# zscole/adversarial-spec

Hardware: AMD Instinct MI355X
Metric: critiques/sec (debate round: 8192-token spec prefill + 512-token critique decode + RCCL consensus all-gather) (higher is better)
Workload: dtype bf16; 1 GPU; model=llama-3-8b, opponents=3, opponents_per_gpu=3, global_batch=3, seq_len=8192, parallelism=opponent-parallel dp1

## Files before the change

### adversarial_spec_amd/models/llama.py

```python

from __future__ import annotations

import math
import os
from dataclasses import dataclass
from typing import Optional

import torch

if torch.cuda.is_available():
    try:
        torch.backends.cuda.preferred_blas_library("cublas")
    except Exception:
        pass

from .. import ops
from ..ops import torch_ref
from .config import LlamaConfig


@dataclass
class QuantW:
    q: torch.Tensor
    s: torch.Tensor
# ... 338 lines not shown

        def proj(x, L_, Qd, name, out):
            qw = Qd.get(name) if Qd is not None else None
            if qw is not None:
                ops.gemv_fp8(x, qw.q, qw.s, W.x8, W.xs, out.view(1, -1))
                return out
            return ops.gemv(x, getattr(L_, name), out=out)

        fused = self.tp is None or self.tp.size == 1
        fused_f8 = (
            fused and fp8 and self.lm_head_q is not None
            and all(
                q.get(f) is not None for q in self.layers_q
                for f in self.FP8_PROJECTIONS
            )
        )

        fused_bf = fused and not fp8

        torch.index_select(self.embed, 0, W.tok_long, out=W.resid)
        if not (fused_bf or fused_f8):
            ops.rmsnorm(W.resid, self.layers[0].attn_norm, c.norm_eps,
                        out=W.normed)
        for i, L in enumerate(self.layers):
            Qd = self.layers_q[i] if fp8 else None
            if fused_f8:
                qw = Qd.get("wqkv")
                if _FP8_LDS:
                    ops.gemv_fp8_norm(W.resid, L.attn_norm, qw.q, qw.s,
                                      c.norm_eps, W.qkv)
                else:
                    ops.quant_norm_fp8(W.resid, L.attn_norm, W.x8, W.xs,
                                       c.norm_eps)
                    ops.gemv_fp8_q(W.x8, W.xs, qw.q, qw.s, W.qkv)
            elif fused_bf:
                ops.gemv_norm(W.resid, L.attn_norm, L.wqkv, c.norm_eps,
                              out=W.qkv)
            else:
                proj(W.normed, L, Qd, "wqkv", W.qkv)
            q = W.qkv[:, : h * hd].view(1, h, hd)
            k = W.qkv[:, h * hd : (h + kh) * hd].view(1, kh, hd)
            v = W.qkv[:, (h + kh) * hd :].view(1, kh, hd)
            ops.rope_kv(q, k, v, self.cos, self.sin, cache.k[i], cache.v[i],
                        cache.page_table, 0, pos_state=pos_state)
            ops.attn_decode_paged(
                q[0], cache.k[i], cache.v[i], cache.page_table,
                max_seq_bound, self.scale, pos_state=pos_state, out=W.attn,
                identity=cache.identity, split_blocks=self.split_blocks,
            )
            if fused_f8:
                gw = Qd.get("w_gate_up")
                if _FP8_LDS:
                    ops.gemv_fp8_resl(W.attn.view(1, h * hd),
                                      Qd.get("wo").q, Qd.get("wo").s,
                                      W.resid)
                    ops.gemv_fp8_gateup_norm(W.resid, L.mlp_norm, gw.q,
                                             gw.s, c.norm_eps, W.act)
                    ops.gemv_fp8_resl(W.act, Qd.get("w_down").q,
                                      Qd.get("w_down").s, W.resid)
                else:
                    ops.gemv_fp8_res(W.attn.view(1, h * hd),
                                     Qd.get("wo").q, Qd.get("wo").s,
                                     W.x8, W.xs, W.resid)
                    ops.quant_norm_fp8(W.resid, L.mlp_norm, W.x8, W.xs,
                                       c.norm_eps)
                    ops.gemv_fp8_gateup(W.x8, W.xs, gw.q, gw.s, W.act)
                    ops.gemv_fp8_res(W.act, Qd.get("w_down").q,
# ... 53 lines not shown
```

### adversarial_spec_amd/ops/__init__.py

```python

from __future__ import annotations

import os
from typing import Optional, Tuple

import torch

from . import torch_ref

_hip = None
_hip_err: Optional[str] = None


def _load_hip():
    global _hip, _hip_err
    if _hip is not None or _hip_err is not None:
        return _hip
    try:
        from . import _advspec_hip

        _hip = _advspec_hip
    except ImportError as e:
        _hip_err = str(e)
    return _hip
# ... 154 lines not shown
    f = w_gate_up.shape[0] // 2
    gu = x @ w_gate_up.t()
    y = torch_ref.swiglu(gu[..., :f], gu[..., f:])
    out.copy_(y.reshape(out.shape))
    return out


def _rms_ref(x: torch.Tensor, eps: float) -> torch.Tensor:
    xf = x.float()
    return torch.rsqrt(xf.pow(2).mean(-1, keepdim=True) + eps)


def gemv_norm(x: torch.Tensor, wln: torch.Tensor, w: torch.Tensor, eps: float,
              out: Optional[torch.Tensor] = None) -> torch.Tensor:
    if _on_gpu(x):
        return _require_hip().gemv_norm(x, wln, w, eps, out)
    y = ((x.float() * _rms_ref(x, eps) * wln.float()) @ w.float().t()).to(x.dtype)
    if out is not None:
        out.copy_(y.reshape(out.shape))
        return out
    return y


def gemv_res(x: torch.Tensor, w: torch.Tensor, resid: torch.Tensor) -> torch.Tensor:
    if _on_gpu(x):
        _require_hip().gemv_res(x, w, resid)
        return resid
    resid.add_((x.float() @ w.float().t()).to(resid.dtype).reshape(resid.shape))
    return resid


def gemv_gateup_norm(x: torch.Tensor, wln: torch.Tensor, w_gate_up: torch.Tensor,
                     eps: float, out: torch.Tensor) -> torch.Tensor:
    if _on_gpu(x):
        _require_hip().gemv_gateup_norm(x, wln, w_gate_up, eps, out)
        return out
    normed = (x.float() * _rms_ref(x, eps) * wln.float()).to(x.dtype)
    return gemv_gateup(normed, w_gate_up, out)


def gemm(x: torch.Tensor, w: torch.Tensor) -> torch.Tensor:
    if _on_gpu(x):
        return _require_hip().gemm(x, w)
    return x @ w.t()


# ... 133 lines not shown
```

### adversarial_spec_amd/ops/hip/attention.hip

```cpp

#include "common.h"

#define MAXG 8

template <int LPP>
DEVINL float group_reduce_sum(float v) {
#pragma unroll
  for (int off = LPP / 2; off > 0; off >>= 1) v += __shfl_xor(v, off, WAVE);
  return v;
}


#define DTILE 64

template <int LPP, int MG, bool IDENT>
__global__ void __launch_bounds__(256) attn_decode_split_kernel(
    const ushort_t *__restrict__ q,
    const ushort_t *__restrict__ kc, const ushort_t *__restrict__ vc,
    const int *__restrict__ page_table, int seq_len, float scale,
    int kh, int group, int hd, int page, int split_len,
    float *__restrict__ ws_m, float *__restrict__ ws_l,
    float *__restrict__ ws_acc, const int *__restrict__ pos_ptr,
    ushort_t *__restrict__ out) {
  if (pos_ptr) seq_len = *pos_ptr + 1;
// ... 157 lines not shown
      if (lane < LPP) {
        const float inv = (l[gi] > 0.f) ? 1.0f / l[gi] : 0.f;
        bf16x8 o;
#pragma unroll
        for (int j = 0; j < 8; ++j) o.u[j] = f32_to_bf16(acc[gi][j] * inv);
        ((bf16x8 *)(out + (size_t)(g * group + gq) * hd))[sl] = o;
      }
    } else {
      const size_t base = ((size_t)g * n_splits + split) * group + gq;
      if (lane == 0) {
        ws_m[base] = m[gi];
        ws_l[base] = l[gi];
      }
      if (lane < LPP) {
#pragma unroll
        for (int j = 0; j < 8; ++j)
          ws_acc[base * hd + sl * 8 + j] = acc[gi][j];
      }
    }
  }
}


extern "C" __global__ void __launch_bounds__(256)
attn_decode_combine_kernel(const float *__restrict__ ws_m,
                           const float *__restrict__ ws_l,
                           const float *__restrict__ ws_acc,
                           ushort_t *__restrict__ out, int n_splits,
                           int group, int hd) {
  const int h = blockIdx.x;
  const int g = h / group, gi = h % group;
  const int dd = blockIdx.y * 64 + (threadIdx.x & (WAVE - 1));
  const int sg = threadIdx.x / WAVE;
  if (dd >= hd) return;

  __shared__ float red[4];
  __shared__ float redL[4];

  float m = -INFINITY;
  {
    float m4[4] = {-INFINITY, -INFINITY, -INFINITY, -INFINITY};
    int s = sg;
    for (; s + 12 < n_splits; s += 16) {
#pragma unroll
      for (int u = 0; u < 4; ++u)
        m4[u] = fmaxf(m4[u],
                      ws_m[((size_t)g * n_splits + s + 4 * u) * group + gi]);
    }
    for (; s < n_splits; s += 4)
      m4[0] = fmaxf(m4[0], ws_m[((size_t)g * n_splits + s) * group + gi]);
    m = fmaxf(fmaxf(m4[0], m4[1]), fmaxf(m4[2], m4[3]));
  }
  if ((threadIdx.x & (WAVE - 1)) == 0) red[sg] = m;
  __syncthreads();
  const float M = fmaxf(fmaxf(red[0], red[1]), fmaxf(red[2], red[3]));

  float L = 0.f, Au[4] = {0.f, 0.f, 0.f, 0.f};
  int s = sg;
  for (; s + 12 < n_splits; s += 16) {
#pragma unroll
    for (int u = 0; u < 4; ++u) {
      const size_t b = ((size_t)g * n_splits + s + 4 * u) * group + gi;
      const float mw = ws_m[b];
      const float sc = (mw == -INFINITY) ? 0.f : exp2f(mw - M);
      L += ws_l[b] * sc;
      Au[u] += ws_acc[b * hd + dd] * sc;
    }
  }
  for (; s < n_splits; s += 4) {
    const size_t b = ((size_t)g * n_splits + s) * group + gi;
    const float mw = ws_m[b];
    const float sc = (mw == -INFINITY) ? 0.f : exp2f(mw - M);
    L += ws_l[b] * sc;
    Au[0] += ws_acc[b * hd + dd] * sc;
  }
  float A = (Au[0] + Au[1]) + (Au[2] + Au[3]);

  __shared__ float accs[4][64];
  accs[sg][threadIdx.x & (WAVE - 1)] = A;
  if ((threadIdx.x & (WAVE - 1)) == 0) redL[sg] = L;
  __syncthreads();
  if (sg == 0) {
    A = accs[0][threadIdx.x] + accs[1][threadIdx.x] + accs[2][threadIdx.x] +
        accs[3][threadIdx.x];
    L = redL[0] + redL[1] + redL[2] + redL[3];
    out[(size_t)h * hd + dd] = f32_to_bf16(L > 0.f ? A / L : 0.f);
  }
}


template <int LPP>
__global__ void __launch_bounds__(256) attn_prefill_simple_kernel(
    const ushort_t *__restrict__ q, const ushort_t *__restrict__ k,
    const ushort_t *__restrict__ v, ushort_t *__restrict__ out,
    int tq, int tk, int kv_offset, float scale, int hq, int kh, int hd,
    int causal) {
  const int h = blockIdx.x;
// ... 110 lines not shown
```

### adversarial_spec_amd/ops/hip/bindings.hip

```cpp

#include <torch/extension.h>
#include <c10/hip/HIPStream.h>
#include <hip/hip_runtime.h>

#include <cstdlib>
#include <mutex>
#include <unordered_map>
#include <vector>

using ushort_t = unsigned short;

extern "C" {
void launch_attn_decode_split(const ushort_t*, const ushort_t*, const ushort_t*,
                              const int*, int, float, int, int, int, int, int,
                              int, float*, float*, float*, const int*,
                              ushort_t*, int, hipStream_t);
void launch_attn_prefill_simple(const ushort_t*, const ushort_t*, const ushort_t*,
                                ushort_t*, int, int, int, float, int, int, int,
                                int, hipStream_t);
void launch_attn_prefill_mfma(const ushort_t*, const ushort_t*, const ushort_t*,
                              ushort_t*, int, int, int, float, int, int, int,
                              hipStream_t, int* ok);
void launch_attn_prefill_mfma_abl(const ushort_t*, const ushort_t*,
                                  const ushort_t*, ushort_t*, int, int, float,
// ... 1 lines not shown
__global__ void mfma_probe_16x16x32(const ushort_t*, const ushort_t*, float*);
__global__ void rmsnorm_kernel(const ushort_t*, const ushort_t*, ushort_t*, int, float);
__global__ void add_rmsnorm_kernel(const ushort_t*, const ushort_t*, const ushort_t*,
                                   ushort_t*, ushort_t*, int, float);
__global__ void rope_kernel(ushort_t*, ushort_t*, const float*, const float*,
                            int, int, int, int, int, long, long, const int*);
__global__ void swiglu_kernel(const ushort_t*, const ushort_t*, ushort_t*, int, int, int);
__global__ void kv_write_kernel(const ushort_t*, const ushort_t*, ushort_t*, ushort_t*,
                                const int*, int, int, int, int, int, const int*);
__global__ void rope_kv_kernel(ushort_t*, ushort_t*, const ushort_t*,
                               const float*, const float*, ushort_t*, ushort_t*,
                               const int*, int, int, int, int, int, long, long,
                               long, int, const int*);
__global__ void sample_kernel(const ushort_t*, int, float, uint32_t, int*);
__global__ void sample_state_kernel(const ushort_t*, int, const float*,
                                    uint32_t*, int*, const int*, long long*);
__global__ void bump_kernel(int*, int*);
void launch_gemv(const ushort_t*, const ushort_t*, ushort_t*, int, int,
                 hipStream_t);
void launch_gemv_gateup(const ushort_t*, const ushort_t*, ushort_t*, int, int,
                        hipStream_t);
void launch_gemv_norm(const ushort_t*, const ushort_t*, const ushort_t*,
                      ushort_t*, int, int, float, hipStream_t);
void launch_gemv_res(const ushort_t*, const ushort_t*, ushort_t*, int, int,
                     hipStream_t);
void launch_gemv_gateup_norm(const ushort_t*, const ushort_t*, const ushort_t*,
                             ushort_t*, int, int, float, hipStream_t);
void launch_gemm(const ushort_t*, const ushort_t*, ushort_t*, int, int, int,
                 hipStream_t);
void launch_gemm256(const ushort_t*, const ushort_t*, ushort_t*, int, int, int,
                    hipStream_t);
void launch_gemm_fp8(const uint8_t*, const float*, const uint8_t*, const float*,
                     ushort_t*, int, int, int, hipStream_t);
void launch_gemm_fp8_256(const uint8_t*, const float*, const uint8_t*,
                         const float*, ushort_t*, int, int, int, hipStream_t);
void launch_quant_norm_fp8(const ushort_t*, const ushort_t*, uint8_t*, float*,
                           int, float, hipStream_t);
void launch_gemv_fp8_norm(const ushort_t*, const ushort_t*, const uint8_t*,
                          const float*, ushort_t*, int, int, float,
                          hipStream_t);
void launch_gemv_fp8_resl(const ushort_t*, const uint8_t*, const float*,
                          ushort_t*, int, int, hipStream_t);
void launch_gemv_fp8_gateup_norm(const ushort_t*, const ushort_t*,
                                 const uint8_t*, const float*, ushort_t*,
                                 int, int, float, hipStream_t);
void launch_gemv_fp8_res(const uint8_t*, const float*, const uint8_t*,
// ... 359 lines not shown

torch::Tensor gemv_norm(torch::Tensor x, torch::Tensor wln, torch::Tensor w,
                        double eps, c10::optional<torch::Tensor> out_opt) {
  CHECK_BF16_CUDA(x);
  CHECK_BF16_CUDA(wln);
  CHECK_BF16_CUDA(w);
  TORCH_CHECK(w.dim() == 2 && w.is_contiguous());
  const int N = w.size(0), K = w.size(1);
  TORCH_CHECK((long)x.numel() == (long)K, "gemv_norm: x numel == K");
  TORCH_CHECK((long)wln.numel() == (long)K, "gemv_norm: wln numel == K");
  TORCH_CHECK(K % 8 == 0, "gemv_norm: K % 8 == 0");
  TORCH_CHECK(K <= 32768, "gemv_norm: LDS xl staging caps K at 32768");
  auto xc = x.contiguous();
  auto lc = wln.contiguous();
  auto y = out_opt.has_value()
               ? *out_opt
               : torch::empty(x.dim() == 2 ? std::vector<int64_t>{1, N}
                                           : std::vector<int64_t>{N},
                              x.options());
  TORCH_CHECK((long)y.numel() == (long)N, "gemv_norm: out numel == N");
  launch_gemv_norm(uptr(xc), uptr(lc), uptr(w), uptr_mut(y), K, N,
                   (float)eps, cur_stream());
  return y;
}

void gemv_res(torch::Tensor x, torch::Tensor w, torch::Tensor resid) {
  CHECK_BF16_CUDA(x);
  CHECK_BF16_CUDA(w);
  CHECK_BF16_CUDA(resid);
  TORCH_CHECK(w.dim() == 2 && w.is_contiguous());
  const int N = w.size(0), K = w.size(1);
  TORCH_CHECK((long)x.numel() == (long)K && K % 8 == 0);
  TORCH_CHECK((long)resid.numel() == (long)N, "gemv_res: resid numel == N");
  TORCH_CHECK(resid.is_contiguous());
  TORCH_CHECK(N <= 8192, "gemv_res: w32 kernel only (hidden <= 8192)");
  auto xc = x.contiguous();
  launch_gemv_res(uptr(xc), uptr(w), uptr_mut(resid), K, N, cur_stream());
}

void gemv_gateup_norm(torch::Tensor x, torch::Tensor wln, torch::Tensor w,
                      double eps, torch::Tensor act) {
  CHECK_BF16_CUDA(x);
  CHECK_BF16_CUDA(wln);
  CHECK_BF16_CUDA(w);
  CHECK_BF16_CUDA(act);
  TORCH_CHECK(w.dim() == 2 && w.is_contiguous());
// ... 311 lines not shown
  m.def("gemm_variant", &gemm_variant, "force GEMM kernel 128/256 (A/B)");
  m.def("gemm_fp8", &gemm_fp8, "fp8 e4m3 MFMA GEMM (rowwise scales)");
  m.def("gemv_fp8", &gemv_fp8, "fp8 decode GEMV (rowwise scales)");
  m.def("quant_norm_fp8", &quant_norm_fp8,
        "fused rmsnorm + rowwise e4m3 quantize (fp8 decode fusion)");
  m.def("gemv_fp8_q", &gemv_fp8_q, "pre-quantized fp8 decode GEMV");
  m.def("gemv_fp8_res", &gemv_fp8_res,
        "fp8 GEMV with residual-add epilogue (fp8 decode fusion)");
  m.def("gemv_fp8_gateup", &gemv_fp8_gateup,
        "pre-quantized fp8 gate_up GEMV + SwiGLU (fp8 decode fusion)");
  m.def("gemv_fp8_norm", &gemv_fp8_norm,
        "rmsnorm + quantize + fp8 GEMV, one launch (LDS-staged)");
  m.def("gemv_fp8_resl", &gemv_fp8_resl,
        "quantize + fp8 GEMV + residual epilogue, one launch (LDS-staged)");
  m.def("gemv_fp8_gateup_norm", &gemv_fp8_gateup_norm,
        "rmsnorm + quantize + fp8 gate_up GEMV + SwiGLU, one launch");
  m.def("quant_fp8", &quant_fp8, "rowwise bf16 -> e4m3 quantizer");
  m.def("mfma_rate", &mfma_rate, "MFMA issue-rate microbench (bf16/fp8)");
  m.def("rope_inplace_ds", &rope_inplace_ds, "graph-mode RoPE (device pos)");
  m.def("rope_kv", &rope_kv, "fused RoPE + paged KV scatter",
        py::arg("q"), py::arg("k"), py::arg("v"), py::arg("cost"),
        py::arg("sint"), py::arg("kc"), py::arg("vc"), py::arg("page_table"),
        py::arg("pos0"), py::arg("pos_state") = py::none());
  m.def("kv_write_ds", &kv_write_ds, "graph-mode KV scatter (device pos)");
  m.def("attn_decode_paged_ds", &attn_decode_paged_ds,
        "graph-mode paged decode attention (device pos)",
        py::arg("q"), py::arg("kc"), py::arg("vc"), py::arg("page_table"),
        py::arg("pos_state"), py::arg("max_seq"), py::arg("scale"),
        py::arg("out") = py::none(), py::arg("identity") = false,
        py::arg("split_blocks") = 0);
  m.def("sample_state", &sample_state, "graph-mode on-device sampling");
  m.def("bump", &bump, "graph-mode pos/step bump");
  m.def("ws_release", &ws_release,
        "drop decode-attention scratch for a dead KV cache");
}
```

### adversarial_spec_amd/ops/hip/common.h

```cpp
#pragma once

#include <hip/hip_runtime.h>
#include <hip/hip_bf16.h>
#include <stdint.h>

#define WAVE 64
#define DEVINL __device__ __forceinline__

typedef unsigned short ushort_t;


DEVINL float bf16_to_f32(ushort_t u) {
  union { uint32_t i; float f; } c;
  c.i = ((uint32_t)u) << 16;
  return c.f;
}

DEVINL ushort_t f32_to_bf16(float f) {
  union { uint32_t i; float f; } c;
  c.f = f;
  uint32_t lsb = (c.i >> 16) & 1u;
  c.i += 0x7fffu + lsb;
  return (ushort_t)(c.i >> 16);
}

struct bf16x8 { ushort_t u[8]; };
struct f32x8  { float v[8]; };

DEVINL f32x8 unpack8(const bf16x8 &p) {
  f32x8 r;
#pragma unroll
  for (int i = 0; i < 8; ++i) r.v[i] = bf16_to_f32(p.u[i]);
  return r;
}

DEVINL bf16x8 pack8(const f32x8 &p) {
  bf16x8 r;
#pragma unroll
  for (int i = 0; i < 8; ++i) r.u[i] = f32_to_bf16(p.v[i]);
  return r;
}

typedef __attribute__((__vector_size__(2 * sizeof(short)))) short bf16x2v_;

DEVINL float dot8_bf16(const bf16x8 &a, const bf16x8 &b, float acc) {
  const bf16x2v_ *ap = (const bf16x2v_ *)&a;
// ... 66 lines not shown
```

### adversarial_spec_amd/ops/hip/elementwise.hip

```cpp

#include "common.h"


extern "C" __global__ void __launch_bounds__(1024)
rmsnorm_kernel(const ushort_t *__restrict__ x, const ushort_t *__restrict__ w,
               ushort_t *__restrict__ y, int d, float eps) {
  __shared__ float scratch[16];
  const int row = blockIdx.x;
  const ushort_t *xr = x + (size_t)row * d;
  ushort_t *yr = y + (size_t)row * d;
  const int nvec = d / 8;

  float ss = 0.f;
  for (int i = threadIdx.x; i < nvec; i += blockDim.x) {
    f32x8 v = unpack8(((const bf16x8 *)xr)[i]);
#pragma unroll
    for (int j = 0; j < 8; ++j) ss += v.v[j] * v.v[j];
  }
  ss = block_reduce_sum(ss, scratch);
  const float inv = rsqrtf(ss / d + eps);

  for (int i = threadIdx.x; i < nvec; i += blockDim.x) {
    f32x8 v = unpack8(((const bf16x8 *)xr)[i]);
    f32x8 ww = unpack8(((const bf16x8 *)w)[i]);
// ... 103 lines not shown
    const int vh = slot - hq - hk;
    const bf16x8 *src =
        (const bf16x8 *)(v + (size_t)tok * v_rstride + (size_t)vh * hd);
    bf16x8 *dst = (bf16x8 *)(vc + cache_row + (size_t)vh * hd);
    for (int i = lane; i < hd / 8; i += WAVE) dst[i] = src[i];
    return;
  }

  const bool is_q = slot < hq;
  ushort_t *base = is_q
                       ? q + (size_t)tok * q_rstride + (size_t)slot * hd
                       : k + (size_t)tok * k_rstride + (size_t)(slot - hq) * hd;
  uint32_t *cache_dst =
      is_q ? nullptr
           : (uint32_t *)(kc + cache_row + (size_t)(slot - hq) * hd);
  const float *crow = cost + (size_t)pos * half;
  const float *srow = sint + (size_t)pos * half;

  for (int p = lane; p < half; p += WAVE) {
    uint32_t pair = ((uint32_t *)base)[p];
    float ev = bf16_to_f32((ushort_t)(pair & 0xffffu));
    float od = bf16_to_f32((ushort_t)(pair >> 16));
    float c = crow[p], s = srow[p];
    const uint32_t rot = (uint32_t)f32_to_bf16(ev * c - od * s) |
                         ((uint32_t)f32_to_bf16(ev * s + od * c) << 16);
    ((uint32_t *)base)[p] = rot;
    if (cache_dst) cache_dst[p] = rot;
  }
}


extern "C" __global__ void __launch_bounds__(256)
swiglu_kernel(const ushort_t *__restrict__ gate, const ushort_t *__restrict__ up,
              ushort_t *__restrict__ out, int t, int f, int in_stride) {
  const size_t nvec = (size_t)t * (f / 8);
  const int fv = f / 8;
  for (size_t i = (size_t)blockIdx.x * blockDim.x + threadIdx.x;
       i < nvec; i += (size_t)gridDim.x * blockDim.x) {
    const size_t row = i / fv, col = i % fv;
    const size_t in_off = row * (in_stride / 8) + col;
    f32x8 g = unpack8(((const bf16x8 *)gate)[in_off]);
    f32x8 u = unpack8(((const bf16x8 *)up)[in_off]);
    f32x8 o;
#pragma unroll
    for (int j = 0; j < 8; ++j) {
      const float gv = g.v[j];
      const float sig = 1.0f / (1.0f + __expf(-gv));
      o.v[j] = gv * sig * u.v[j];
// ... 29 lines not shown
```

### adversarial_spec_amd/ops/hip/gemm_fp8.hip

```cpp

#include "common.h"

typedef __attribute__((__vector_size__(4 * sizeof(float)))) float f32x4v;
typedef __attribute__((__vector_size__(2 * sizeof(float)))) float f32x2v;

DEVINL float dot16_fp8(const uint4 &xv, const uint4 &wv) {
  const int *x32 = (const int *)&xv;
  const int *w32 = (const int *)&wv;
  float acc = 0.f;
#pragma unroll
  for (int q = 0; q < 4; ++q) {
    const f32x2v xl = __builtin_amdgcn_cvt_pk_f32_fp8(x32[q], false);
    const f32x2v xh = __builtin_amdgcn_cvt_pk_f32_fp8(x32[q], true);
    const f32x2v wl = __builtin_amdgcn_cvt_pk_f32_fp8(w32[q], false);
    const f32x2v wh = __builtin_amdgcn_cvt_pk_f32_fp8(w32[q], true);
    acc += xl[0] * wl[0] + xl[1] * wl[1] + xh[0] * wh[0] + xh[1] * wh[1];
  }
  return acc;
}

#define F8_M 128
#define F8_N 128
#define F8_K 64

// ... 305 lines not shown
  const int nc = K / 16;

  float acc = 0.f;
  int c = sl;
  for (; c + 96 < nc; c += 128) {
    uint4 wv[4], xv[4];
#pragma unroll
    for (int u = 0; u < 4; ++u) {
      wv[u] = *(const uint4 *)(wr + (size_t)(c + 32 * u) * 16);
      xv[u] = *(const uint4 *)(x + (size_t)(c + 32 * u) * 16);
    }
#pragma unroll
    for (int u = 0; u < 4; ++u) acc += dot16_fp8(xv[u], wv[u]);
  }
  for (; c < nc; c += 32) {
    const uint4 wv = *(const uint4 *)(wr + (size_t)c * 16);
    const uint4 xv = *(const uint4 *)(x + (size_t)c * 16);
    acc += dot16_fp8(xv, wv);
  }

#pragma unroll
  for (int off = 16; off > 0; off >>= 1) acc += __shfl_xor(acc, off, WAVE);
  if (sl == 0) y[n] = f32_to_bf16(acc * xs[0] * wsc[n]);
}

extern "C" void launch_gemv_fp8(const uint8_t *x, const float *xs,
                                const uint8_t *w, const float *wsc,
                                ushort_t *y, int K, int N,
                                hipStream_t stream) {
  if (N <= 8192) {
    gemv_fp8_kernel_w32<<<dim3((N + 7) / 8), 256, 0, stream>>>(x, xs, w, wsc,
                                                               y, K, N);
  } else {
    gemv_fp8_kernel<<<dim3((N + 15) / 16), 256, 0, stream>>>(x, xs, w, wsc, y,
                                                             K, N);
  }
}

extern "C" void launch_quant_fp8(const ushort_t *x, uint8_t *q, float *scale,
                                 int M, int K, hipStream_t stream) {
  quant_fp8_row_kernel<<<dim3(M), 256, 0, stream>>>(x, q, scale, K);
}


extern "C" __global__ void __launch_bounds__(256)
quant_norm_fp8_kernel(const ushort_t *__restrict__ x,
// ... 375 lines not shown
```

### adversarial_spec_amd/ops/hip/gemv.hip

```cpp

#include "common.h"

DEVINL float group16_sum(float v) {
#pragma unroll
  for (int off = 8; off > 0; off >>= 1) v += __shfl_xor(v, off, WAVE);
  return v;
}

extern "C" __global__ void __launch_bounds__(256)
gemv_kernel(const ushort_t *__restrict__ x, const ushort_t *__restrict__ w,
            ushort_t *__restrict__ y, int K, int N) {
  const int lane = threadIdx.x & (WAVE - 1);
  const int wid = threadIdx.x / WAVE;
  const int rg = lane >> 4;
  const int sl = lane & 15;
  const int n = blockIdx.x * 16 + wid * 4 + rg;
  if (n >= N) return;

  const ushort_t *wr = w + (size_t)n * K;
  const int nc = K / 8;

  float acc = 0.f;
  int c = sl;
  for (; c + 48 < nc; c += 64) {
// ... 150 lines not shown
  const int n0 = blockIdx.x * 8 + wid * 2 + rg;
  const int n = n0 < N ? n0 : N - 1;

  const float rms = norm_stage_lds(x, wln, xl, red, K, eps);

  const ushort_t *wr = w + (size_t)n * K;
  const int nc = K / 8;
  float acc = 0.f;
  int c = sl;
  for (; c + 224 < nc; c += 256) {
    bf16x8 wv[8];
#pragma unroll
    for (int u = 0; u < 8; ++u) wv[u] = ((const bf16x8 *)wr)[c + 32 * u];
#pragma unroll
    for (int u = 0; u < 8; ++u)
      acc = dot8_bf16(((const bf16x8 *)xl)[c + 32 * u], wv[u], acc);
  }
  for (; c < nc; c += 32)
    acc = dot8_bf16(((const bf16x8 *)xl)[c], ((const bf16x8 *)wr)[c], acc);

#pragma unroll
  for (int off = 16; off > 0; off >>= 1) acc += __shfl_xor(acc, off, WAVE);
  if (sl == 0 && n0 < N) y[n0] = f32_to_bf16(acc * rms);
}

extern "C" __global__ void __launch_bounds__(256)
gemv_norm_kernel(const ushort_t *__restrict__ x,
                 const ushort_t *__restrict__ wln,
                 const ushort_t *__restrict__ w,
                 ushort_t *__restrict__ y, int K, int N, float eps) {
  extern __shared__ ushort_t xl[];
  __shared__ float red[16];
  const int lane = threadIdx.x & (WAVE - 1);
  const int wid = threadIdx.x / WAVE;
  const int rg = lane >> 4;
  const int sl = lane & 15;
  const int n0 = blockIdx.x * 16 + wid * 4 + rg;
  const int n = n0 < N ? n0 : N - 1;

  const float rms = norm_stage_lds(x, wln, xl, red, K, eps);

  const ushort_t *wr = w + (size_t)n * K;
  const int nc = K / 8;
  float acc = 0.f;
  int c = sl;
  for (; c + 48 < nc; c += 64) {
// ... 94 lines not shown
    ag += __shfl_xor(ag, off, WAVE);
    au += __shfl_xor(au, off, WAVE);
  }
  if (sl == 0 && n0 < F) {
    const float g = ag * rms;
    const float s = g / (1.0f + __expf(-g));
    act[n0] = f32_to_bf16(s * (au * rms));
  }
}

extern "C" void launch_gemv_norm(const ushort_t *x, const ushort_t *wln,
                                 const ushort_t *w, ushort_t *y, int K, int N,
                                 float eps, hipStream_t stream) {
  const size_t lds = (size_t)K * 2;
  if (N <= 8192)
    gemv_norm_w32_kernel<<<dim3((N + 7) / 8), 256, lds, stream>>>(x, wln, w,
                                                                  y, K, N,
                                                                  eps);
  else
    gemv_norm_kernel<<<dim3((N + 15) / 16), 256, lds, stream>>>(x, wln, w, y,
                                                                K, N, eps);
}

extern "C" void launch_gemv_res(const ushort_t *x, const ushort_t *w,
                                ushort_t *resid, int K, int N,
                                hipStream_t stream) {
  gemv_res_w32_kernel<<<dim3((N + 7) / 8), 256, 0, stream>>>(x, w, resid, K, N);
}

extern "C" void launch_gemv_gateup_norm(const ushort_t *x, const ushort_t *wln,
                                        const ushort_t *w, ushort_t *act,
                                        int K, int F, float eps,
                                        hipStream_t stream) {
  gemv_gateup_norm_kernel<<<dim3((F + 7) / 8), 256, (size_t)K * 2, stream>>>(
      x, wln, w, act, K, F, eps);
}
```

Baseline: 0.5874 critiques/s.

## Fuse RoPE and KV-cache write into QKV GEMV epilogue for decode

Adds bf16 and fp8 QKV GEMV kernels whose epilogue pairs adjacent output rows across wave halves, applies the rotary rotation, and writes K/V straight into the paged cache. This removes the separate rope_kv launch and its re-read of the QKV buffer every layer during decode. It also restructures the split-attention combine kernel to prefetch all split partials into registers when there are at most 64 splits. The rounding of the rotation is pinned with contract-off blocks so results match the old path. In exchange the fused path runs on a w32 geometry with 8 rows per block, capped at N <= 8192.

```diff
diff --git a/adversarial_spec_amd/models/llama.py b/adversarial_spec_amd/models/llama.py
--- a/adversarial_spec_amd/models/llama.py
+++ b/adversarial_spec_amd/models/llama.py
@@ -384,8 +384,11 @@
         if not (fused_bf or fused_f8):
             ops.rmsnorm(W.resid, self.layers[0].attn_norm, c.norm_eps,
                         out=W.normed)
+        fuse_rope = ops.qkv_rope_fusable(h, kh, hd, self.cos, self.sin,
+                                         cache.k[0], cache.v[0])
         for i, L in enumerate(self.layers):
             Qd = self.layers_q[i] if fp8 else None
+            roped = False
             if fused_f8:
                 qw = Qd.get("wqkv")
                 if _FP8_LDS:
@@ -394,17 +397,33 @@
                 else:
                     ops.quant_norm_fp8(W.resid, L.attn_norm, W.x8, W.xs,
                                        c.norm_eps)
-                    ops.gemv_fp8_q(W.x8, W.xs, qw.q, qw.s, W.qkv)
+                    if fuse_rope:
+                        ops.gemv_fp8_q_rope_kv(
+                            W.x8, W.xs, qw.q, qw.s, W.qkv, self.cos, self.sin,
+                            cache.k[i], cache.v[i], cache.page_table, 0, h,
+                            kh, pos_state=pos_state)
+                        roped = True
+                    else:
+                        ops.gemv_fp8_q(W.x8, W.xs, qw.q, qw.s, W.qkv)
             elif fused_bf:
-                ops.gemv_norm(W.resid, L.attn_norm, L.wqkv, c.norm_eps,
-                              out=W.qkv)
+                if fuse_rope:
+                    ops.gemv_norm_rope_kv(
+                        W.resid, L.attn_norm, L.wqkv, c.norm_eps, self.cos,
+                        self.sin, cache.k[i], cache.v[i], cache.page_table, 0,
+                        h, kh, pos_state=pos_state, out=W.qkv)
+                    roped = True
+                else:
+                    ops.gemv_norm(W.resid, L.attn_norm, L.wqkv, c.norm_eps,
+                                  out=W.qkv)
             else:
                 proj(W.normed, L, Qd, "wqkv", W.qkv)
             q = W.qkv[:, : h * hd].view(1, h, hd)
-            k = W.qkv[:, h * hd : (h + kh) * hd].view(1, kh, hd)
-            v = W.qkv[:, (h + kh) * hd :].view(1, kh, hd)
-            ops.rope_kv(q, k, v, self.cos, self.sin, cache.k[i], cache.v[i],
-                        cache.page_table, 0, pos_state=pos_state)
+            if not roped:
+                k = W.qkv[:, h * hd : (h + kh) * hd].view(1, kh, hd)
+                v = W.qkv[:, (h + kh) * hd :].view(1, kh, hd)
+                ops.rope_kv(q, k, v, self.cos, self.sin, cache.k[i],
+                            cache.v[i], cache.page_table, 0,
+                            pos_state=pos_state)
             ops.attn_decode_paged(
                 q[0], cache.k[i], cache.v[i], cache.page_table,
                 max_seq_bound, self.scale, pos_state=pos_state, out=W.attn,
diff --git a/adversarial_spec_amd/ops/__init__.py b/adversarial_spec_amd/ops/__init__.py
--- a/adversarial_spec_amd/ops/__init__.py
+++ b/adversarial_spec_amd/ops/__init__.py
@@ -200,6 +200,88 @@
     return y
 
 
+def qkv_rope_fusable(hq: int, kh: int, hd: int,
+                     cos: Optional[torch.Tensor] = None,
+                     sin: Optional[torch.Tensor] = None,
+                     k_cache: Optional[torch.Tensor] = None,
+                     v_cache: Optional[torch.Tensor] = None) -> bool:
+    if hd % 16 != 0 or (hq + 2 * kh) * hd > 8192:
+        return False
+    for t in (cos, sin):
+        if t is not None and not (
+            t.dtype == torch.float32 and t.dim() == 2 and t.is_contiguous()
+            and t.shape[1] == hd // 2
+        ):
+            return False
+    if cos is not None and sin is not None and cos.shape != sin.shape:
+        return False
+    for t in (k_cache, v_cache):
+        if t is not None and not (
+            t.dtype == torch.bfloat16 and t.dim() == 4 and t.is_contiguous()
+            and t.shape[2] == kh and t.shape[3] == hd
+        ):
+            return False
+    if (k_cache is not None and v_cache is not None
+            and k_cache.shape != v_cache.shape):
+        return False
+    return True
+
+
+def _rope_kv_on_qkv(y: torch.Tensor, hq: int, kh: int, cos, sin, k_cache,
+                    v_cache, page_table, pos0: int, pos_state) -> torch.Tensor:
+    hd = y.numel() // (hq + 2 * kh)
+    if pos_state is not None:
+        pos0 = int(pos_state.reshape(-1)[0])
+    row = y.view(1, -1)
+    q = row[:, : hq * hd].view(1, hq, hd)
+    k = row[:, hq * hd : (hq + kh) * hd].view(1, kh, hd)
+    v = row[:, (hq + kh) * hd :].view(1, kh, hd)
+    q2, k2 = rope_kv(q, k, v, cos, sin, k_cache, v_cache, page_table, pos0)
+    q.copy_(q2)
+    k.copy_(k2)
+    return y
+
+
+def gemv_norm_rope_kv(
+    x: torch.Tensor, wln: torch.Tensor, w: torch.Tensor, eps: float,
+    cos: torch.Tensor, sin: torch.Tensor, k_cache: torch.Tensor,
+    v_cache: torch.Tensor, page_table: torch.Tensor, pos0: int,
+    hq: int, kh: int, pos_state: Optional[torch.Tensor] = None,
+    out: Optional[torch.Tensor] = None,
+) -> torch.Tensor:
+    if _on_gpu(x):
+        return _require_hip().gemv_norm_rope_kv(
+            x, wln, w, eps, cos, sin, k_cache, v_cache, page_table, pos0,
+            hq, kh, pos_state, out)
+    y = gemv_norm(x, wln, w, eps).reshape(1, -1).contiguous()
+    _rope_kv_on_qkv(y, hq, kh, cos, sin, k_cache, v_cache, page_table, pos0,
+                    pos_state)
+    if out is not None:
+        out.copy_(y.reshape(out.shape))
+        return out
+    return y
+
+
+def gemv_fp8_q_rope_kv(
+    x8: torch.Tensor, xs: torch.Tensor, w_q: torch.Tensor,
+    w_scale: torch.Tensor, out: torch.Tensor, cos: torch.Tensor,
+    sin: torch.Tensor, k_cache: torch.Tensor, v_cache: torch.Tensor,
+    page_table: torch.Tensor, pos0: int, hq: int, kh: int,
+    pos_state: Optional[torch.Tensor] = None,
+) -> torch.Tensor:
+    if x8.is_cuda:
+        _require_hip().gemv_fp8_q_rope_kv(
+            x8, xs, w_q, w_scale, out, cos, sin, k_cache, v_cache,
+            page_table, pos0, hq, kh, pos_state)
+        return out
+    y = torch.empty(1, w_q.shape[0], dtype=out.dtype)
+    gemv_fp8_q(x8, xs, w_q, w_scale, y)
+    _rope_kv_on_qkv(y, hq, kh, cos, sin, k_cache, v_cache, page_table, pos0,
+                    pos_state)
+    out.copy_(y.reshape(out.shape))
+    return out
+
+
 def gemv_res(x: torch.Tensor, w: torch.Tensor, resid: torch.Tensor) -> torch.Tensor:
     if _on_gpu(x):
         _require_hip().gemv_res(x, w, resid)
diff --git a/adversarial_spec_amd/ops/hip/attention.hip b/adversarial_spec_amd/ops/hip/attention.hip
--- a/adversarial_spec_amd/ops/hip/attention.hip
+++ b/adversarial_spec_amd/ops/hip/attention.hip
@@ -203,6 +203,21 @@
 }
 
 
+DEVINL void combine_step_round(float &L, float &A, float l, float a,
+                               float sc) {
+  {
+#pragma clang fp contract(off)
+    L = L + l * sc;
+  }
+  A = __builtin_fmaf(a, sc, A);
+}
+
+DEVINL void combine_step_ragged(float &L, float &A, float l, float a,
+                                float sc) {
+  L = __builtin_fmaf(l, sc, L);
+  A = __builtin_fmaf(a, sc, A);
+}
+
 extern "C" __global__ void __launch_bounds__(256)
 attn_decode_combine_kernel(const float *__restrict__ ws_m,
                            const float *__restrict__ ws_l,
@@ -218,42 +233,80 @@
   __shared__ float red[4];
   __shared__ float redL[4];
 
-  float m = -INFINITY;
-  {
+  float L = 0.f, Au[4] = {0.f, 0.f, 0.f, 0.f};
+  if (n_splits <= 64) {
+    float mw[16], lw[16], aw[16];
+#pragma unroll
+    for (int j = 0; j < 16; ++j) {
+      const int sc = min(sg + 4 * j, n_splits - 1);
+      const size_t b = ((size_t)g * n_splits + sc) * group + gi;
+      mw[j] = ws_m[b];
+      lw[j] = ws_l[b];
+      aw[j] = ws_acc[b * hd + dd];
+    }
     float m4[4] = {-INFINITY, -INFINITY, -INFINITY, -INFINITY};
+#pragma unroll
+    for (int j = 0; j < 16; ++j)
+      if (sg + 4 * j < n_splits) m4[j & 3] = fmaxf(m4[j & 3], mw[j]);
+    const float m = fmaxf(fmaxf(m4[0], m4[1]), fmaxf(m4[2], m4[3]));
+    if ((threadIdx.x & (WAVE - 1)) == 0) red[sg] = m;
+    __syncthreads();
+    const float M = fmaxf(fmaxf(red[0], red[1]), fmaxf(red[2], red[3]));
+#pragma unroll
+    for (int r = 0; r < 4; ++r) {
+      if (sg + 16 * r + 12 < n_splits) {
+#pragma unroll
+        for (int u = 0; u < 4; ++u) {
+          const int j = 4 * r + u;
+          const float sc = (mw[j] == -INFINITY) ? 0.f : exp2f(mw[j] - M);
+          combine_step_round(L, Au[u], lw[j], aw[j], sc);
+        }
+      } else {
+#pragma unroll
+        for (int u = 0; u < 4; ++u) {
+          const int j = 4 * r + u;
+          if (sg + 4 * j < n_splits) {
+            const float sc = (mw[j] == -INFINITY) ? 0.f : exp2f(mw[j] - M);
+            combine_step_ragged(L, Au[0], lw[j], aw[j], sc);
+          }
+        }
+      }
+    }
+  } else {
+    float m = -INFINITY;
+    {
+      float m4[4] = {-INFINITY, -INFINITY, -INFINITY, -INFINITY};
+      int s = sg;
+      for (; s + 12 < n_splits; s += 16) {
+#pragma unroll
+        for (int u = 0; u < 4; ++u)
+          m4[u] = fmaxf(m4[u],
+                        ws_m[((size_t)g * n_splits + s + 4 * u) * group + gi]);
+      }
+      for (; s < n_splits; s += 4)
+        m4[0] = fmaxf(m4[0], ws_m[((size_t)g * n_splits + s) * group + gi]);
+      m = fmaxf(fmaxf(m4[0], m4[1]), fmaxf(m4[2], m4[3]));
+    }
+    if ((threadIdx.x & (WAVE - 1)) == 0) red[sg] = m;
+    __syncthreads();
+    const float M = fmaxf(fmaxf(red[0], red[1]), fmaxf(red[2], red[3]));
+
     int s = sg;
     for (; s + 12 < n_splits; s += 16) {
 #pragma unroll
-      for (int u = 0; u < 4; ++u)
-        m4[u] = fmaxf(m4[u],
-                      ws_m[((size_t)g * n_splits + s + 4 * u) * group + gi]);
-    }
-    for (; s < n_splits; s += 4)
-      m4[0] = fmaxf(m4[0], ws_m[((size_t)g * n_splits + s) * group + gi]);
-    m = fmaxf(fmaxf(m4[0], m4[1]), fmaxf(m4[2], m4[3]));
-  }
-  if ((threadIdx.x & (WAVE - 1)) == 0) red[sg] = m;
-  __syncthreads();
-  const float M = fmaxf(fmaxf(red[0], red[1]), fmaxf(red[2], red[3]));
-
-  float L = 0.f, Au[4] = {0.f, 0.f, 0.f, 0.f};
-  int s = sg;
-  for (; s + 12 < n_splits; s += 16) {
-#pragma unroll
-    for (int u = 0; u < 4; ++u) {
-      const size_t b = ((size_t)g * n_splits + s + 4 * u) * group + gi;
+      for (int u = 0; u < 4; ++u) {
+        const size_t b = ((size_t)g * n_splits + s + 4 * u) * group + gi;
+        const float mw = ws_m[b];
+        const float sc = (mw == -INFINITY) ? 0.f : exp2f(mw - M);
+        combine_step_round(L, Au[u], ws_l[b], ws_acc[b * hd + dd], sc);
+      }
+    }
+    for (; s < n_splits; s += 4) {
+      const size_t b = ((size_t)g * n_splits + s) * group + gi;
       const float mw = ws_m[b];
       const float sc = (mw == -INFINITY) ? 0.f : exp2f(mw - M);
-      L += ws_l[b] * sc;
-      Au[u] += ws_acc[b * hd + dd] * sc;
-    }
-  }
-  for (; s < n_splits; s += 4) {
-    const size_t b = ((size_t)g * n_splits + s) * group + gi;
-    const float mw = ws_m[b];
-    const float sc = (mw == -INFINITY) ? 0.f : exp2f(mw - M);
-    L += ws_l[b] * sc;
-    Au[0] += ws_acc[b * hd + dd] * sc;
+      combine_step_ragged(L, Au[0], ws_l[b], ws_acc[b * hd + dd], sc);
+    }
   }
   float A = (Au[0] + Au[1]) + (Au[2] + Au[3]);
 
diff --git a/adversarial_spec_amd/ops/hip/bindings.hip b/adversarial_spec_amd/ops/hip/bindings.hip
--- a/adversarial_spec_amd/ops/hip/bindings.hip
+++ b/adversarial_spec_amd/ops/hip/bindings.hip
@@ -47,6 +47,15 @@
                         hipStream_t);
 void launch_gemv_norm(const ushort_t*, const ushort_t*, const ushort_t*,
                       ushort_t*, int, int, float, hipStream_t);
+void launch_gemv_norm_rope_kv(const ushort_t*, const ushort_t*,
+                              const ushort_t*, ushort_t*, int, float,
+                              const float*, const float*, ushort_t*, ushort_t*,
+                              const int*, const int*, int, int, int, int, int,
+                              hipStream_t);
+void launch_gemv_fp8_rope_kv(const uint8_t*, const float*, const uint8_t*,
+                             const float*, ushort_t*, int, const float*,
+                             const float*, ushort_t*, ushort_t*, const int*,
+                             const int*, int, int, int, int, int, hipStream_t);
 void launch_gemv_res(const ushort_t*, const ushort_t*, ushort_t*, int, int,
                      hipStream_t);
 void launch_gemv_gateup_norm(const ushort_t*, const ushort_t*, const ushort_t*,
@@ -452,6 +461,113 @@
   launch_gemv_norm(uptr(xc), uptr(lc), uptr(w), uptr_mut(y), K, N,
                    (float)eps, cur_stream());
   return y;
+}
+
+struct RopeKvGeom { int hd, page; const int* pos_ptr; };
+static RopeKvGeom check_rope_kv_epilogue(
+    const char* op, int N, int64_t hq, int64_t kh, const torch::Tensor& cost,
+    const torch::Tensor& sint, const torch::Tensor& kc,
+    const torch::Tensor& vc, const torch::Tensor& page_table, int64_t pos0,
+    const c10::optional<torch::Tensor>& pos_state, const torch::Tensor& y) {
+  TORCH_CHECK(hq >= 1 && kh >= 1 && N % (hq + 2 * kh) == 0, op,
+              ": N == (hq + 2*kh)*hd");
+  const int hd = N / (int)(hq + 2 * kh);
+  TORCH_CHECK(hd % 16 == 0, op, ": hd % 16 == 0");
+  TORCH_CHECK(N <= 8192, op, ": w32 geometry only (N <= 8192)");
+  TORCH_CHECK(cost.is_cuda() && sint.is_cuda() &&
+                  cost.scalar_type() == at::kFloat &&
+                  sint.scalar_type() == at::kFloat,
+              op, ": cos/sin tables f32 on GPU");
+  TORCH_CHECK(cost.dim() == 2 && cost.is_contiguous() &&
+                  sint.is_contiguous() && cost.sizes() == sint.sizes() &&
+                  cost.size(1) == hd / 2,
+              op, ": cos/sin tables [max_pos, hd/2] contiguous");
+  CHECK_BF16_CUDA(kc);
+  CHECK_BF16_CUDA(vc);
+  TORCH_CHECK(kc.is_contiguous() && vc.is_contiguous(), op,
+              ": caches contiguous");
+  TORCH_CHECK(kc.dim() == 4 && kc.sizes() == vc.sizes() && kc.size(2) == kh &&
+                  kc.size(3) == hd,
+              op, ": caches [n_pages, page, kh, hd]");
+  TORCH_CHECK(page_table.is_cuda() && page_table.scalar_type() == at::kInt &&
+                  page_table.is_contiguous(),
+              op, ": page_table int32 on GPU");
+  const int page = kc.size(1);
+  const int* pp = nullptr;
+  if (pos_state.has_value()) {
+    TORCH_CHECK(pos_state->is_cuda() && pos_state->scalar_type() == at::kInt &&
+                    pos_state->numel() >= 1,
+                op, ": pos_state int32 word on GPU");
+    pp = pos_state->data_ptr<int>();
+  } else {
+    TORCH_CHECK(pos0 >= 0 && pos0 < cost.size(0) &&
+                    pos0 / page < page_table.numel(),
+                op, ": pos inside the rope table and the page table");
+  }
+  CHECK_BF16_CUDA(y);
+  TORCH_CHECK(y.is_contiguous() && (long)y.numel() == (long)N, op,
+              ": out contiguous, numel == N");
+  TORCH_CHECK(reinterpret_cast<uintptr_t>(y.data_ptr()) % 4 == 0, op,
+              ": out 4-byte aligned (pairs are stored as one word)");
+  return {hd, page, pp};
+}
+
+torch::Tensor gemv_norm_rope_kv(
+    torch::Tensor x, torch::Tensor wln, torch::Tensor w, double eps,
+    torch::Tensor cost, torch::Tensor sint, torch::Tensor kc, torch::Tensor vc,
+    torch::Tensor page_table, int64_t pos0, int64_t hq, int64_t kh,
+    const c10::optional<torch::Tensor>& pos_state,
+    c10::optional<torch::Tensor> out_opt) {
+  CHECK_BF16_CUDA(x);
+  CHECK_BF16_CUDA(wln);
+  CHECK_BF16_CUDA(w);
+  TORCH_CHECK(w.dim() == 2 && w.is_contiguous());
+  const int N = w.size(0), K = w.size(1);
+  TORCH_CHECK((long)x.numel() == (long)K, "gemv_norm_rope_kv: x numel == K");
+  TORCH_CHECK((long)wln.numel() == (long)K,
+              "gemv_norm_rope_kv: wln numel == K");
+  TORCH_CHECK(K % 8 == 0, "gemv_norm_rope_kv: K % 8 == 0");
+  TORCH_CHECK(K <= 32768, "gemv_norm_rope_kv: LDS xl staging caps K at 32768");
+  auto xc = x.contiguous();
+  auto lc = wln.contiguous();
+  auto y = out_opt.has_value() ? *out_opt : torch::empty({1, N}, x.options());
+  const RopeKvGeom g = check_rope_kv_epilogue(
+      "gemv_norm_rope_kv", N, hq, kh, cost, sint, kc, vc, page_table, pos0,
+      pos_state, y);
+  launch_gemv_norm_rope_kv(uptr(xc), uptr(lc), uptr(w), uptr_mut(y), K,
+                           (float)eps, cost.data_ptr<float>(),
+                           sint.data_ptr<float>(), uptr_mut(kc), uptr_mut(vc),
+                           page_table.data_ptr<int>(), g.pos_ptr, (int)pos0,
+                           (int)hq, (int)kh, g.hd, g.page, cur_stream());
+  return y;
+}
+
+void gemv_fp8_q_rope_kv(torch::Tensor x8, torch::Tensor xs, torch::Tensor w8,
+                        torch::Tensor wsc, torch::Tensor out,
+                        torch::Tensor cost, torch::Tensor sint,
+                        torch::Tensor kc, torch::Tensor vc,
+                        torch::Tensor page_table, int64_t pos0, int64_t hq,
+                        int64_t kh,
+                        const c10::optional<torch::Tensor>& pos_state) {
+  TORCH_CHECK(w8.dim() == 2 && w8.is_contiguous() && w8.is_cuda() &&
+              w8.scalar_type() == at::kByte);
+  const int N = w8.size(0), K = w8.size(1);
+  TORCH_CHECK(K % 16 == 0, "gemv_fp8_q_rope_kv: K % 16 == 0");
+  TORCH_CHECK(x8.is_cuda() && x8.numel() >= K &&
+              x8.scalar_type() == at::kByte && x8.is_contiguous());
+  TORCH_CHECK(xs.is_cuda() && xs.numel() >= 1 &&
+              xs.scalar_type() == at::kFloat);
+  TORCH_CHECK(wsc.is_cuda() && wsc.numel() >= N &&
+              wsc.scalar_type() == at::kFloat && wsc.is_contiguous());
+  const RopeKvGeom g = check_rope_kv_epilogue(
+      "gemv_fp8_q_rope_kv", N, hq, kh, cost, sint, kc, vc, page_table, pos0,
+      pos_state, out);
+  launch_gemv_fp8_rope_kv(x8.data_ptr<uint8_t>(), xs.data_ptr<float>(),
+                          w8.data_ptr<uint8_t>(), wsc.data_ptr<float>(),
+                          uptr_mut(out), K, cost.data_ptr<float>(),
+                          sint.data_ptr<float>(), uptr_mut(kc), uptr_mut(vc),
+                          page_table.data_ptr<int>(), g.pos_ptr, (int)pos0,
+                          (int)hq, (int)kh, g.hd, g.page, cur_stream());
 }
 
 void gemv_res(torch::Tensor x, torch::Tensor w, torch::Tensor resid) {
@@ -809,6 +925,18 @@
         py::arg("q"), py::arg("k"), py::arg("v"), py::arg("cost"),
         py::arg("sint"), py::arg("kc"), py::arg("vc"), py::arg("page_table"),
         py::arg("pos0"), py::arg("pos_state") = py::none());
+  m.def("gemv_norm_rope_kv", &gemv_norm_rope_kv,
+        "rmsnorm + qkv GEMV + RoPE + KV append, one launch (decode fusion)",
+        py::arg("x"), py::arg("wln"), py::arg("w"), py::arg("eps"),
+        py::arg("cost"), py::arg("sint"), py::arg("kc"), py::arg("vc"),
+        py::arg("page_table"), py::arg("pos0"), py::arg("hq"), py::arg("kh"),
+        py::arg("pos_state") = py::none(), py::arg("out") = py::none());
+  m.def("gemv_fp8_q_rope_kv", &gemv_fp8_q_rope_kv,
+        "pre-quantized fp8 qkv GEMV + RoPE + KV append, one launch",
+        py::arg("x8"), py::arg("xs"), py::arg("w8"), py::arg("wsc"),
+        py::arg("out"), py::arg("cost"), py::arg("sint"), py::arg("kc"),
+        py::arg("vc"), py::arg("page_table"), py::arg("pos0"), py::arg("hq"),
+        py::arg("kh"), py::arg("pos_state") = py::none());
   m.def("kv_write_ds", &kv_write_ds, "graph-mode KV scatter (device pos)");
   m.def("attn_decode_paged_ds", &attn_decode_paged_ds,
         "graph-mode paged decode attention (device pos)",
diff --git a/adversarial_spec_amd/ops/hip/common.h b/adversarial_spec_amd/ops/hip/common.h
--- a/adversarial_spec_amd/ops/hip/common.h
+++ b/adversarial_spec_amd/ops/hip/common.h
@@ -22,6 +22,18 @@
   uint32_t lsb = (c.i >> 16) & 1u;
   c.i += 0x7fffu + lsb;
   return (ushort_t)(c.i >> 16);
+}
+
+DEVINL uint32_t rope_rotate_pair(float ev, float od, float c, float s) {
+  float od_s, od_c;
+  {
+#pragma clang fp contract(off)
+    od_s = od * s;
+    od_c = od * c;
+  }
+  const float e2 = __builtin_fmaf(ev, c, -od_s);
+  const float o2 = __builtin_fmaf(ev, s, od_c);
+  return (uint32_t)f32_to_bf16(e2) | ((uint32_t)f32_to_bf16(o2) << 16);
 }
 
 struct bf16x8 { ushort_t u[8]; };
diff --git a/adversarial_spec_amd/ops/hip/elementwise.hip b/adversarial_spec_amd/ops/hip/elementwise.hip
--- a/adversarial_spec_amd/ops/hip/elementwise.hip
+++ b/adversarial_spec_amd/ops/hip/elementwise.hip
@@ -149,8 +149,7 @@
     float ev = bf16_to_f32((ushort_t)(pair & 0xffffu));
     float od = bf16_to_f32((ushort_t)(pair >> 16));
     float c = crow[p], s = srow[p];
-    const uint32_t rot = (uint32_t)f32_to_bf16(ev * c - od * s) |
-                         ((uint32_t)f32_to_bf16(ev * s + od * c) << 16);
+    const uint32_t rot = rope_rotate_pair(ev, od, c, s);
     ((uint32_t *)base)[p] = rot;
     if (cache_dst) cache_dst[p] = rot;
   }
diff --git a/adversarial_spec_amd/ops/hip/gemm_fp8.hip b/adversarial_spec_amd/ops/hip/gemm_fp8.hip
--- a/adversarial_spec_amd/ops/hip/gemm_fp8.hip
+++ b/adversarial_spec_amd/ops/hip/gemm_fp8.hip
@@ -1,5 +1,6 @@
 
 #include "common.h"
+#include "rope_epilogue.h"
 
 typedef __attribute__((__vector_size__(4 * sizeof(float)))) float f32x4v;
 typedef __attribute__((__vector_size__(2 * sizeof(float)))) float f32x2v;
@@ -351,6 +352,60 @@
 #pragma unroll
   for (int off = 16; off > 0; off >>= 1) acc += __shfl_xor(acc, off, WAVE);
   if (sl == 0) y[n] = f32_to_bf16(acc * xs[0] * wsc[n]);
+}
+
+extern "C" __global__ void __launch_bounds__(256)
+gemv_fp8_rope_kv_w32_kernel(const uint8_t *__restrict__ x,
+                            const float *__restrict__ xs,
+                            const uint8_t *__restrict__ w,
+                            const float *__restrict__ wsc,
+                            ushort_t *__restrict__ y, int K, RopeKvArgs ra) {
+  const int lane = threadIdx.x & (WAVE - 1);
+  const int wid = threadIdx.x / WAVE;
+  const int rg = lane >> 5;
+  const int sl = lane & 31;
+  const int n_even = blockIdx.x * 8 + wid * 2;
+  const int n = n_even + rg;
+
+  const RopeKvPre pre = rope_kv_prefetch(ra, n_even);
+  const float ws_n = wsc[n];
+
+  const uint8_t *wr = w + (size_t)n * K;
+  const int nc = K / 16;
+
+  float acc = 0.f;
+  int c = sl;
+  for (; c + 96 < nc; c += 128) {
+    uint4 wv[4], xv[4];
+#pragma unroll
+    for (int u = 0; u < 4; ++u) {
+      wv[u] = *(const uint4 *)(wr + (size_t)(c + 32 * u) * 16);
+      xv[u] = *(const uint4 *)(x + (size_t)(c + 32 * u) * 16);
+    }
+#pragma unroll
+    for (int u = 0; u < 4; ++u) acc += dot16_fp8(xv[u], wv[u]);
+  }
+  for (; c < nc; c += 32) {
+    const uint4 wv = *(const uint4 *)(wr + (size_t)c * 16);
+    const uint4 xv = *(const uint4 *)(x + (size_t)c * 16);
+    acc += dot16_fp8(xv, wv);
+  }
+
+#pragma unroll
+  for (int off = 16; off > 0; off >>= 1) acc += __shfl_xor(acc, off, WAVE);
+  rope_kv_store(pre, y, n_even, acc * xs[0] * ws_n, lane);
+}
+
+extern "C" void launch_gemv_fp8_rope_kv(
+    const uint8_t *x, const float *xs, const uint8_t *w, const float *wsc,
+    ushort_t *y, int K, const float *cost, const float *sint, ushort_t *kc,
+    ushort_t *vc, const int *page_table, const int *pos_ptr, int pos, int hq,
+    int kh, int hd, int page, hipStream_t stream) {
+  const int N = (hq + 2 * kh) * hd;
+  const RopeKvArgs ra = {cost, sint, kc, vc, page_table, pos_ptr,
+                         pos,  hq,   kh, hd, page};
+  gemv_fp8_rope_kv_w32_kernel<<<dim3(N / 8), 256, 0, stream>>>(x, xs, w, wsc,
+                                                               y, K, ra);
 }
 
 extern "C" void launch_gemv_fp8(const uint8_t *x, const float *xs,
diff --git a/adversarial_spec_amd/ops/hip/gemv.hip b/adversarial_spec_amd/ops/hip/gemv.hip
--- a/adversarial_spec_amd/ops/hip/gemv.hip
+++ b/adversarial_spec_amd/ops/hip/gemv.hip
@@ -1,5 +1,6 @@
 
 #include "common.h"
+#include "rope_epilogue.h"
 
 DEVINL float group16_sum(float v) {
 #pragma unroll
@@ -196,6 +197,45 @@
 #pragma unroll
   for (int off = 16; off > 0; off >>= 1) acc += __shfl_xor(acc, off, WAVE);
   if (sl == 0 && n0 < N) y[n0] = f32_to_bf16(acc * rms);
+}
+
+extern "C" __global__ void __launch_bounds__(256)
+gemv_norm_rope_kv_w32_kernel(const ushort_t *__restrict__ x,
+                             const ushort_t *__restrict__ wln,
+                             const ushort_t *__restrict__ w,
+                             ushort_t *__restrict__ y, int K, float eps,
+                             RopeKvArgs ra) {
+  extern __shared__ ushort_t xl[];
+  __shared__ float red[16];
+  const int lane = threadIdx.x & (WAVE - 1);
+  const int wid = threadIdx.x / WAVE;
+  const int rg = lane >> 5;
+  const int sl = lane & 31;
+  const int n_even = blockIdx.x * 8 + wid * 2;
+  const int n = n_even + rg;
+
+  const RopeKvPre pre = rope_kv_prefetch(ra, n_even);
+
+  const float rms = norm_stage_lds(x, wln, xl, red, K, eps);
+
+  const ushort_t *wr = w + (size_t)n * K;
+  const int nc = K / 8;
+  float acc = 0.f;
+  int c = sl;
+  for (; c + 224 < nc; c += 256) {
+    bf16x8 wv[8];
+#pragma unroll
+    for (int u = 0; u < 8; ++u) wv[u] = ((const bf16x8 *)wr)[c + 32 * u];
+#pragma unroll
+    for (int u = 0; u < 8; ++u)
+      acc = dot8_bf16(((const bf16x8 *)xl)[c + 32 * u], wv[u], acc);
+  }
+  for (; c < nc; c += 32)
+    acc = dot8_bf16(((const bf16x8 *)xl)[c], ((const bf16x8 *)wr)[c], acc);
+
+#pragma unroll
+  for (int off = 16; off > 0; off >>= 1) acc += __shfl_xor(acc, off, WAVE);
+  rope_kv_store(pre, y, n_even, acc * rms, lane);
 }
 
 extern "C" __global__ void __launch_bounds__(256)
@@ -336,6 +376,18 @@
                                                                 K, N, eps);
 }
 
+extern "C" void launch_gemv_norm_rope_kv(
+    const ushort_t *x, const ushort_t *wln, const ushort_t *w, ushort_t *y,
+    int K, float eps, const float *cost, const float *sint, ushort_t *kc,
+    ushort_t *vc, const int *page_table, const int *pos_ptr, int pos, int hq,
+    int kh, int hd, int page, hipStream_t stream) {
+  const int N = (hq + 2 * kh) * hd;
+  const RopeKvArgs ra = {cost, sint, kc, vc, page_table, pos_ptr,
+                         pos,  hq,   kh, hd, page};
+  gemv_norm_rope_kv_w32_kernel<<<dim3(N / 8), 256, (size_t)K * 2, stream>>>(
+      x, wln, w, y, K, eps, ra);
+}
+
 extern "C" void launch_gemv_res(const ushort_t *x, const ushort_t *w,
                                 ushort_t *resid, int K, int N,
                                 hipStream_t stream) {
diff --git a/adversarial_spec_amd/ops/hip/rope_epilogue.h b/adversarial_spec_amd/ops/hip/rope_epilogue.h
--- /dev/null
+++ b/adversarial_spec_amd/ops/hip/rope_epilogue.h
@@ -0,0 +1,54 @@
+#pragma once
+
+#include "common.h"
+
+struct RopeKvArgs {
+  const float *cost, *sint;
+  ushort_t *kc, *vc;
+  const int *page_table;
+  const int *pos_ptr;
+  int pos;
+  int hq, kh, hd, page;
+};
+
+struct RopeKvPre {
+  float c, s;
+  ushort_t *cache;
+  bool rotate;
+};
+
+DEVINL RopeKvPre rope_kv_prefetch(const RopeKvArgs &a, int n_even) {
+  const int pos = a.pos_ptr ? *a.pos_ptr : a.pos;
+  const int half = a.hd / 2;
+  const int slot = n_even / a.hd;
+  const int d = n_even - slot * a.hd;
+  const int phys = a.page_table[pos / a.page];
+  const size_t cache_row =
+      ((size_t)phys * a.page + (pos % a.page)) * a.kh * a.hd;
+  RopeKvPre r;
+  r.c = a.cost[(size_t)pos * half + (d >> 1)];
+  r.s = a.sint[(size_t)pos * half + (d >> 1)];
+  r.rotate = slot < a.hq + a.kh;
+  if (slot < a.hq)
+    r.cache = nullptr;
+  else if (r.rotate)
+    r.cache = a.kc + cache_row + (size_t)(slot - a.hq) * a.hd + d;
+  else
+    r.cache = a.vc + cache_row + (size_t)(slot - a.hq - a.kh) * a.hd + d;
+  return r;
+}
+
+DEVINL void rope_kv_store(const RopeKvPre &pre, ushort_t *__restrict__ y,
+                          int n_even, float val, int lane) {
+  const uint32_t mine = f32_to_bf16(val);
+  const uint32_t other = (uint32_t)__shfl_xor((int)mine, 32, WAVE);
+  if (lane != 0) return;
+  uint32_t pair = mine | (other << 16);
+  if (pre.rotate) {
+    const float ev = bf16_to_f32((ushort_t)mine);
+    const float od = bf16_to_f32((ushort_t)other);
+    pair = rope_rotate_pair(ev, od, pre.c, pre.s);
+  }
+  *(uint32_t *)(y + n_even) = pair;
+  if (pre.cache) *(uint32_t *)pre.cache = pair;
+}
```

Result: faster. 0.6029 critiques/s (median of 6 runs) (+2.6%).
